# andrewdalpino/UltraZoom

Hardware: AMD Instinct MI355X
Metric: upscaled MPix/sec, MewZoom-4X 1080p bf16 batched inference (higher is better)
Workload: dtype bf16; 1 GPU; MewZoom-4X 96ch/40L bf16, 16 x 1080x1920 -> 4320x7680 per GPU; global_batch=16, parallelism=batch-sharded x1, images_in_flight=0

## Files before the change

ultrazoom_amd/csrc/mz_conv3r.h:

```cpp
#pragma once
#include "mz_device.h"
#include "mz_diag.h"
#include "mz_relay.h"

namespace mz {
namespace r3 {

constexpr int TH = 8;
template <int GEO> struct Geo {
    static_assert(GEO == 0 || GEO == 1, "8 x 48 or 8 x 40");
    static constexpr int TW = GEO == 0 ? 48 : 40;
    static constexpr int NPF = GEO == 0 ? 6 : 5;
    static constexpr int ROWW = TW + 2;
    static constexpr int NPIX = 10 * ROWW;
    static constexpr int DIV_MAGIC = GEO == 0 ? 1311 : 1561;
    static constexpr int X0 = 3, X1 = NPF - 3;
    static constexpr bool straddle(int pf) { return GEO == 1 && pf == 2; }
    static constexpr int dy(int pf) { return GEO == 0 ? pf / 3 : (pf >= 3 ? 1 : 0); }
    static constexpr int dx(int pf) { return GEO == 0 ? 16 * (pf % 3) : (pf < 2 ? 16 * pf : (pf == 2 ? 0 : 8 + 16 * (pf - 3))); }
};
constexpr int PLANE_ENT = 512;
constexpr int A_PLANE = PLANE_ENT * 16;
constexpr int A_SLOT = 4 * A_PLANE;
constexpr int NT = 3, NF = 6, BN = 96;
constexpr int NG = 9 * NT;
constexpr int B_BASE = 2 * A_SLOT;
constexpr int CHUNK_PIECES = 2 * NG;
constexpr int MIX_PIECES = 4 * NT * NT;

template <int NSEG> struct Seg {
    static_assert(NSEG == 2 || NSEG == 3, "two or three weight segments per chunk");
    static constexpr int start(int s) { return NSEG == 2 ? (s <= 0 ? 0 : (s == 1 ? (NG + 1) / 2 : NG)) : (NG / 3) * s; }
    static constexpr int of(int G) { return NSEG == 2 ? (G < start(1) ? 0 : 1) : G / (NG / 3); }
    static constexpr int pieces(int s) { return 2 * (start(s + 1) - start(s)); }
    static constexpr int SLOT = pieces(0) * 1024;
    static constexpr int MIX_BASE = B_BASE + 3 * SLOT;
    static constexpr int lds_bytes(bool fuse) { return fuse ? MIX_BASE + MIX_PIECES * 1024 : B_BASE + 3 * SLOT; }
};

template <int GEO, int TAP, int PF> constexpr int a_off() {
    using GG = Geo<GEO>;
    constexpr int DY = TAP / 3, DX = TAP % 3;
    return ((DY + GG::dy(PF)) * GG::ROWW + DX + GG::dx(PF)) * 16;
}

template <int NPF> struct Frag {
    u32x4 x[2][NPF];
    u32x4 w[3][2];
};

template <int N> __device__ __forceinline__ void wait_w(u32x4& w0, u32x4& w1) {
    asm volatile("s_waitcnt lgkmcnt(%2)" : "+v"(w0), "+v"(w1) : "n"(N) : "memory");
}
template <int N>
__device__ __forceinline__ void wait_wx(u32x4& w0, u32x4& w1, u32x4 (&x)[6]) {
    asm volatile("s_waitcnt lgkmcnt(%8)"
                 : "+v"(w0), "+v"(w1), "+v"(x[0]), "+v"(x[1]), "+v"(x[2]), "+v"(x[3]), "+v"(x[4]), "+v"(x[5])
                 : "n"(N)
                 : "memory");
}
template <int N>
__device__ __forceinline__ void wait_wx(u32x4& w0, u32x4& w1, u32x4 (&x)[5]) {
    asm volatile("s_waitcnt lgkmcnt(%7)"
                 : "+v"(w0), "+v"(w1), "+v"(x[0]), "+v"(x[1]), "+v"(x[2]), "+v"(x[3]), "+v"(x[4])
                 : "n"(N)
                 : "memory");
}

struct Bases {
    uint32_t a_cur, a_nxt, b_cur, b_nxt;
    uint32_t a2_cur, a2_nxt;
};
template <int GEO, int TAP, int PF> __device__ __forceinline__ u32x4 read_x(const Bases& bs, const bool next_image) {
    if constexpr (Geo<GEO>::straddle(PF)) return lds_read128<a_off<GEO, TAP, PF>()>(next_image ? bs.a2_nxt : bs.a2_cur);
    else return lds_read128<a_off<GEO, TAP, PF>()>(next_image ? bs.a_nxt : bs.a_cur);
}

template <class TT, int NSEG, int GEO, int GC, int XP, bool ZERO_C, int M>
__device__ __forceinline__ void group_mfmas(f32x4 (&acc)[Geo<GEO>::NPF][NF], Frag<Geo<GEO>::NPF>& f, const Bases& bs) {
    using GG = Geo<GEO>;
    constexpr int NPF = GG::NPF;
    if constexpr (M < 2 * NPF) {
        using S = Seg<NSEG>;
        constexpr int t = GC / 3, n = GC % 3, xp = (t + XP) & 1, xq = xp ^ 1;
        constexpr int sg = S::of(GC);
        constexpr int Gs = S::start(sg), Ge = S::start(sg + 1);
        constexpr int T = GC + 2;
        constexpr bool t_here = T < Ge;
        constexpr int t_idx = t_here ? T - Gs : T - Ge;
        constexpr int pf = (n & 1) ? NPF - 1 - M / 2 : M / 2, k = ((M / 2) & 1) ? 1 - (M & 1) : (M & 1);
        if constexpr (ZERO_C) mma16_first<TT>(acc[pf][2 * n + k], f.w[GC % 3][k], f.x[xp][pf]);
        else mma16<TT>(acc[pf][2 * n + k], f.w[GC % 3][k], f.x[xp][pf]);
        __builtin_amdgcn_sched_barrier(0);
        if constexpr (M < 2) {
            f.w[T % 3][M] = lds_read128<(2 * t_idx + M) * 1024>(t_here ? bs.b_cur : bs.b_nxt);
            __builtin_amdgcn_sched_barrier(0);
        }
        if constexpr (n < 2 && M >= 2 && M < 2 + (n == 0 ? GG::X0 : GG::X1)) {
            constexpr int pfn = GG::X0 * n + (M - 2);
            if constexpr (t + 1 < 9) f.x[xq][pfn] = read_x<GEO, (t + 1 < 9 ? t + 1 : 0), pfn>(bs, false);
            else f.x[xq][pfn] = read_x<GEO, 0, pfn>(bs, true);
            __builtin_amdgcn_sched_barrier(0);
        }
        group_mfmas<TT, NSEG, GEO, GC, XP, ZERO_C, M + 1>(acc, f, bs);
    }
}

template <class TT, int NSEG, int GEO, int G, int GE, int XP>
__device__ __forceinline__ void groups(f32x4 (&acc)[Geo<GEO>::NPF][NF], Frag<Geo<GEO>::NPF>& f, const Bases& bs, bool first) {
    using GG = Geo<GEO>;
    if constexpr (G < GE) {
        constexpr int t = G / 3, n = G % 3;
        __builtin_amdgcn_sched_barrier(0);
        if constexpr (G < 3 && XP == 0) {
            if (first) group_mfmas<TT, NSEG, GEO, G, XP, true, 0>(acc, f, bs);
            else group_mfmas<TT, NSEG, GEO, G, XP, false, 0>(acc, f, bs);
        } else {
            group_mfmas<TT, NSEG, GEO, G, XP, false, 0>(acc, f, bs);
        }
        constexpr int wn = (G + 1) % 3, xn = (t + 1 + XP) & 1;
        if constexpr (n == 2)
            wait_wx<2>(f.w[wn][0], f.w[wn][1], f.x[xn]);
        else if constexpr (n == 1)
            wait_w<GG::X0 + 2 + GG::X1>(f.w[wn][0], f.w[wn][1]);
        else
            wait_w<2 + GG::X0>(f.w[wn][0], f.w[wn][1]);
        groups<TT, NSEG, GEO, G + 1, GE, XP>(acc, f, bs, first);
    }
}

template <int H, int I> __device__ __forceinline__ void gate_reads(u32x4 (&wv)[NT], uint32_t addr) {
    if constexpr (I < NT) {
        constexpr int ks = H >> 1, part = H & 1;
        wv[I] = lds_read128<(ks * 2 * NT + part * NT + I) * 1024>(addr);
        gate_reads<H, I + 1>(wv, addr);
    }
}
template <int N> __device__ __forceinline__ void gate_wait(u32x4 (&wv)[NT]) {
    asm volatile("s_waitcnt lgkmcnt(%3)" : "+v"(wv[0]), "+v"(wv[1]), "+v"(wv[2]) : "n"(N) : "memory");
}
template <class TT, int H>
__device__ __forceinline__ void gate_halves(f32x4 (&beta)[NF], const u32x4 (&xf)[NT], const u32x4 (&zf)[NT], u32x4 (&wa)[NT],
                                            u32x4 (&wb)[NT], uint32_t addr) {
    if constexpr (H < 4 * NT) {
        constexpr int ks = H >> 1, part = H & 1;
        constexpr bool more = H + 1 < 4 * NT;
        if constexpr (more) gate_reads<H + 1, 0>(wb, addr);
        gate_wait<(more ? NT : 0)>(wa);
        __builtin_amdgcn_sched_barrier(0);
#pragma unroll
        for (int i = 0; i < NT; ++i) {
            if constexpr (ks == 0) mma16_first<TT>(beta[part * NT + i], wa[i], xf[0]);
            else if constexpr (ks < NT) mma16<TT>(beta[part * NT + i], wa[i], xf[ks]);
            else mma16<TT>(beta[part * NT + i], wa[i], zf[ks - NT]);
        }
        __builtin_amdgcn_sched_barrier(0);
        gate_halves<TT, H + 1>(beta, xf, zf, wb, wa, addr);
    }
}

}

template <class TT, int NSEG, int EPI, bool SILU, int GEO = 0, bool RAG = false>
__global__ __launch_bounds__(512) void conv3r_kernel(const ConvArgs a) {
    using namespace r3;
    using namespace relay;
    using S = Seg<NSEG>;
    using GG = Geo<GEO>;
    constexpr int NPF = GG::NPF, TW = GG::TW, ROWW = GG::ROWW, NPIX = GG::NPIX;
    constexpr int NE = NPF * NT;
    constexpr bool FUSE = EPI == EPI_FUSEDMIX;
    static_assert(!FUSE || GEO == 0, "the fused variant is built for the 8 x 48 tile");
    constexpr int B_SLOT = S::SLOT;
    static_assert(!FUSE || NSEG == 3, "the gate weights need the LDS that three weight segments leave free");
    static_assert(!RAG || (NSEG == 3 && EPI == EPI_STORE && GEO == 0), "the ragged two-chunk variant: three steps per chunk, plain stores, 8 x 48 tiles");
    extern __shared__ __attribute__((aligned(16))) char smem[];
    const int w = __builtin_amdgcn_readfirstlane((int)threadIdx.x >> 6);
    const int team = w >> 2, wq = w & 3;
    const int nchunks = a.nchunks16;
    const uint32_t lds_base = (uint32_t)(uintptr_t)(__attribute__((address_space(3))) char*)smem;

    const int xcd = blockIdx.x & 7, pos = blockIdx.x >> 3, step = gridDim.x >> 3;
    const int q = a.grid >> 3, rem = a.grid & 7;
    const int cnt = q + (xcd < rem ? 1 : 0);
    const int base = xcd < rem ? xcd * (q + 1) : rem * (q + 1) + (xcd - rem) * q;
    if (pos >= cnt) return;
    typedef uint32_t TabE __attribute__((ext_vector_type(2)));
    typedef const __attribute__((address_space(4))) TabE* TabPtr;
    const TabPtr tab = (TabPtr)(uintptr_t)a.tile_tab + base;
    struct TileE { uint32_t yx, bn; };
    auto tile_at = [&](int i) __attribute__((always_inline)) {
        const TabE e = tab[i];
        return TileE{e[0], e[1]};
    };
    int a_pos = pos;
    TileE eD, eA, eB;
    auto advance = [&]() __attribute__((always_inline)) { a_pos += step; };
    auto tile_origin = [&](const TileE e, int& b, int& y0, int& x0) __attribute__((always_inline)) {
        b = (int)(e.bn & 0xffffu);
        y0 = (int)(e.yx & 0xffffu);
        x0 = (int)(e.yx >> 16);
    };
    auto tile_nt = [](const TileE e) __attribute__((always_inline)) { return (int)(e.bn >> 16); };

    int hs = 0, us = 0;
    auto next3 = [](int v) __attribute__((always_inline)) { return v == 2 ? 0 : v + 1; };

    f32x4 acc[NPF][NF];
    Frag<NPF> f;
    RS_DECL;

    const size_t chunk_bytes = (size_t)CHUNK_PIECES * 1024;
    const long long plane_in = (long long)a.H * a.W * 16;

    uint32_t hoff[2];
    const char* img_l = nullptr;
    auto set_load_tile = [&](const TileE e) __attribute__((always_inline)) {
        int b, y0, x0;
        tile_origin(e, b, y0, x0);
        img_l = (const char*)a.in0 + (long long)b * a.p0 * plane_in;
        const int lane_ = lane_now();
        const bool interior = y0 >= 1 && x0 >= 1 && y0 + TH + 2 <= a.H && x0 + TW + 1 <= a.W;
        const uint32_t delta = ((uint32_t)(y0 - 1) * (uint32_t)a.W + (uint32_t)(x0 - 1)) * 16u;
#pragma unroll
        for (int j = 0; j < 2; ++j) {
            const int p = 64 * (wq + 4 * j) + lane_;
            const int py = (p * GG::DIV_MAGIC) >> 16, px = p - py * ROWW;
            uint32_t o = ((uint32_t)py * (uint32_t)a.W + (uint32_t)px) * 16u + delta;
            if (!interior) {
                const int gy = y0 - 1 + py, gx = x0 - 1 + px;
                const bool ok = (p < NPIX) & (gy >= 0) & (gy < a.H) & (gx >= 0) & (gx < a.W);
                o = ok ? o : 0xffffffffu;
            }
            hoff[j] = o;
        }
    };
    auto halo_piece = [&](auto i_tag, const __amdgpu_buffer_rsrc_t rsrc, char* dst, [[maybe_unused]] const bool rag = false) __attribute__((always_inline)) {
        constexpr int i = decltype(i_tag)::value;
        uint32_t off = hoff[i & 1];
        if constexpr (RAG) {
            if (rag && (i >> 1) >= a.ragged_planes) off = 0xffffffffu;
        }
        __builtin_amdgcn_raw_ptr_buffer_load_lds(rsrc, (__attribute__((address_space(3))) void*)(dst + (wq + 4 * i) * 1024), 16,
                                                 (int)off, (int)((uint32_t)(i >> 1) * (uint32_t)plane_in), 0, 0);
    };
    auto halo_rsrc = [&](int kc) __attribute__((always_inline)) {
        return __builtin_amdgcn_make_buffer_rsrc((void*)(img_l + 4LL * kc * plane_in), 0, (int)(uint32_t)(4 * plane_in), 0x00020000);
    };
    auto wseg_count = [&](int pieces) __attribute__((always_inline)) { return pieces > wq ? (pieces - wq + 3) >> 2 : 0; };
    auto wseg_piece = [&](auto i_tag, const char* s0, int mine, char* dst, uint32_t lo) __attribute__((always_inline)) {
        constexpr int i = decltype(i_tag)::value;
        if (i < mine) glds16(s0 + (size_t)wq * 1024u + (size_t)i * 4096u + lo, dst + wq * 1024 + i * 4096);
    };
    constexpr int WP = (S::pieces(0) + 3) / 4;
    auto wsrc_of = [&](int nt) __attribute__((always_inline)) {
        return (const char*)a.wpk16 + (size_t)nt * nchunks * chunk_bytes;
    };

    __amdgpu_buffer_rsrc_t orsrc;
    u32x4 xrsrc = {0u, 0u, 0u, 0u};
    uint32_t x_lane = 0;
    uint32_t e_pix = 0, eoff[NT] = {0, 0, 0};
    int e_c = 0, e_y = 0;
    [[maybe_unused]] int e_sdy = 0, e_sdx = 0;
    [[maybe_unused]] uint32_t e_soff = 0;
    auto epi_setup = [&]() __attribute__((always_inline)) {
        const int lane_ = lane_now();
        const int g = lane_ >> 4, c = lane_ & 15;
        const int lane_cu = 2 * (g & 1) + (g >> 1);
        int d_b, d_y0, d_x0;
        tile_origin(eD, d_b, d_y0, d_x0);
        const int d_nbase = tile_nt(eD) * BN;
        e_c = d_x0 + c;
        e_y = d_y0 + 2 * wq;
        if constexpr (GEO == 1) {
            e_sdy = c >= 8 ? 1 : 0;
            e_sdx = c >= 8 ? -8 : 32;
        }
        if constexpr (EPI == EPI_D2S) {
            const long long plane_o = (long long)a.Hout * a.Wout * 16;
            orsrc = __builtin_amdgcn_make_buffer_rsrc((char*)a.out + (long long)d_b * a.p_out * plane_o, 0,
                                                      (int)(uint32_t)(a.p_out * plane_o), 0x00020000);
            e_pix = ((uint32_t)(2 * e_y) * (uint32_t)a.Wout + (uint32_t)(2 * e_c)) * 16u;
            if constexpr (GEO == 1) e_soff = (uint32_t)((2 * e_sdy * a.Wout + 2 * e_sdx) * 16);
#pragma unroll
            for (int n = 0; n < NT; ++n) {
                const int nch = d_nbase + (4 * n + lane_cu) * 8;
                const int ij = nch / a.cp_out, ch = nch - ij * a.cp_out;
                eoff[n] = nch < 4 * a.cp_out
                              ? (uint32_t)(ch >> 3) * (uint32_t)plane_o + ((uint32_t)(ij >> 1) * (uint32_t)a.Wout + (uint32_t)(ij & 1)) * 16u
                              : 0xffffffffu;
            }
        } else {
            const long long plane_o = (long long)a.H * a.W * 16;
            const int p_first = d_nbase >> 3;
            const int planes = a.p_out - p_first < 4 * NT ? a.p_out - p_first : 4 * NT;
            orsrc = __builtin_amdgcn_make_buffer_rsrc((char*)a.out + ((long long)d_b * a.p_out + p_first) * plane_o, 0,
                                                      (int)(uint32_t)(planes * plane_o), 0x00020000);
            e_pix = ((uint32_t)e_y * (uint32_t)a.W + (uint32_t)e_c) * 16u;
            if constexpr (GEO == 1) e_soff = (uint32_t)((e_sdy * a.W + e_sdx) * 16);
#pragma unroll
            for (int n = 0; n < NT; ++n) eoff[n] = (uint32_t)(4 * n + lane_cu) * (uint32_t)plane_o;
            if constexpr (FUSE) {
                const unsigned long long xb = (unsigned long long)(uintptr_t)((const char*)a.in1 + (long long)d_b * a.p1 * plane_o);
                xrsrc[0] = (uint32_t)__builtin_amdgcn_readfirstlane((int)(uint32_t)xb);
                xrsrc[1] = (uint32_t)__builtin_amdgcn_readfirstlane((int)(uint32_t)((xb >> 32) & 0xffffu));
                xrsrc[2] = (uint32_t)__builtin_amdgcn_readfirstlane((int)(uint32_t)(a.p1 * plane_o));
                xrsrc[3] = 0x00020000u;
                x_lane = (uint32_t)(g >> 1) * (uint32_t)plane_o + (uint32_t)(g & 1) * 8u;
            }
        }
    };
    typedef uint32_t u32x2_ __attribute__((ext_vector_type(2)));
    u32x2_ f_xq[2][NF];
    u32x4 f_zb[NT];
    auto entry_words = [&](auto e_tag, u32x4& o) __attribute__((always_inline)) {
        constexpr int E = decltype(e_tag)::value;
        constexpr int pf = E / NT, n = E % NT;
        uint32_t pa[2], pb[2];
#pragma unroll
        for (int h = 0; h < 2; ++h) {
            float a0 = acc[pf][2 * n][2 * h], a1 = acc[pf][2 * n][2 * h + 1], b0 = acc[pf][2 * n + 1][2 * h], b1 = acc[pf][2 * n + 1][2 * h + 1];
            if constexpr (FUSE) {
                float xa[2], za[2], xc[2], zc[2];
                unpack2r<TT>(f_xq[pf & 1][2 * n][h], xa[0], xa[1]);
                unpack2r<TT>(f_zb[n][h], za[0], za[1]);
                unpack2r<TT>(f_xq[pf & 1][2 * n + 1][h], xc[0], xc[1]);
                unpack2r<TT>(f_zb[n][2 + h], zc[0], zc[1]);
                blend_pair_to(a0, a1, acc[pf][2 * n][2 * h], acc[pf][2 * n][2 * h + 1], xa[0], xa[1], za[0], za[1], a.inv_mix_scale);
                blend_pair_to(b0, b1, acc[pf][2 * n + 1][2 * h], acc[pf][2 * n + 1][2 * h + 1], xc[0], xc[1], zc[0], zc[1], a.inv_mix_scale);
            }
            if constexpr (EPI == EPI_STORE && SILU) {
                silu_pair_to(a0, a1, acc[pf][2 * n][2 * h], acc[pf][2 * n][2 * h + 1]);
                silu_pair_to(b0, b1, acc[pf][2 * n + 1][2 * h], acc[pf][2 * n + 1][2 * h + 1]);
            }
            pa[h] = pack_pair<TT>(f32x2{a0, a1});
            pb[h] = pack_pair<TT>(f32x2{b0, b1});
        }
        o = swap_packed(pa, pb);
    };
    auto epi_store = [&](auto e_tag, const u32x4& o) __attribute__((always_inline)) {
        constexpr int E = decltype(e_tag)::value;
        constexpr int pf = E / NT, n = E % NT;
        bool inside;
        uint32_t off;
        if constexpr (GG::straddle(pf)) {
            inside = e_y + e_sdy < a.H && e_c + e_sdx < a.W;
            off = e_pix + e_soff + eoff[n];
        } else {
            inside = e_y + GG::dy(pf) < a.H && e_c + GG::dx(pf) < a.W;
            if constexpr (EPI == EPI_D2S) off = e_pix + (uint32_t)(2 * GG::dy(pf)) * (uint32_t)a.Wout * 16u + (uint32_t)(2 * GG::dx(pf)) * 16u + eoff[n];
            else off = e_pix + (uint32_t)GG::dy(pf) * (uint32_t)a.W * 16u + (uint32_t)GG::dx(pf) * 16u + eoff[n];
        }
        if (!inside || eoff[n] == 0xffffffffu) off = 0xffffffffu;
        __builtin_amdgcn_raw_buffer_store_b128(o, orsrc, (int)off, 0, 0);
    };
    auto fuse_x = [&](auto pf_tag) __attribute__((always_inline)) {
        constexpr int pf = decltype(pf_tag)::value;
        const bool inside = e_y + GG::dy(pf) < a.H && e_c + GG::dx(pf) < a.W;
        const long long plane_o = (long long)a.H * a.W * 16;
        uint32_t off = e_pix + (uint32_t)GG::dy(pf) * (uint32_t)a.W * 16u + (uint32_t)GG::dx(pf) * 16u + x_lane;
        if (!inside) off = 0xffffffffu;
#pragma unroll
        for (int nf = 0; nf < NF; ++nf) {
            const uint32_t o = inside ? off + (uint32_t)(2 * nf) * (uint32_t)plane_o : 0xffffffffu;
            u32x2_& dst = f_xq[pf & 1][nf];
            const u32x4& xr = xrsrc;
            asm volatile("buffer_load_dwordx2 %0, %1, %2, 0 offen" : "=v"(dst) : "v"(o), "s"(xr) : "memory");
        }
    };
    auto x_landed = [&](auto pf_tag) __attribute__((always_inline)) {
        constexpr int pf = decltype(pf_tag)::value;
#pragma unroll
        for (int nf = 0; nf < NF; ++nf) {
            u32x2_& r = f_xq[pf & 1][nf];
            asm volatile("" : "+v"(r));
        }
    };
    auto fuse_z = [&](auto pf_tag) __attribute__((always_inline)) {
        constexpr int pf = decltype(pf_tag)::value;
#pragma unroll
        for (int m = 0; m < NT; ++m) {
            const f32x4 za = acc[pf][2 * m], zc = acc[pf][2 * m + 1];
            u32x4 q;
            q[0] = pack2r<TT>(za[0], za[1]); q[1] = pack2r<TT>(za[2], za[3]);
            q[2] = pack2r<TT>(zc[0], zc[1]); q[3] = pack2r<TT>(zc[2], zc[3]);
            asm volatile("" : "+v"(q));
            f_zb[m] = q;
        }
    };
    auto fuse_a = [&](auto pf_tag) __attribute__((always_inline)) {
        constexpr int pf = decltype(pf_tag)::value;
        if constexpr (pf + 1 < NPF) fuse_x(ic<(pf + 1 < NPF ? pf + 1 : 0)>{});
        fuse_z(pf_tag);
    };
    auto fuse_c = [&](auto pf_tag) __attribute__((always_inline)) {
        constexpr int pf = decltype(pf_tag)::value;
        const int lane_ = lane_now();
        const uint32_t mix_lane = lds_base + S::MIX_BASE + lane_ * 16;
        u32x4 xb[NT];
#pragma unroll
        for (int m = 0; m < NT; ++m) xb[m] = u32x4{f_xq[pf & 1][2 * m][0], f_xq[pf & 1][2 * m][1], f_xq[pf & 1][2 * m + 1][0], f_xq[pf & 1][2 * m + 1][1]};
        u32x4 wa[NT], wb[NT];
        gate_reads<0, 0>(wa, mix_lane);
        gate_halves<TT, 0>(acc[pf], xb, f_zb, wa, wb, mix_lane);
        gate_settle();
    };
    auto entry_whole = [&](auto e_tag) __attribute__((always_inline)) {
        if constexpr (decltype(e_tag)::value < NE) {
            u32x4 o;
            entry_words(e_tag, o);
            epi_store(e_tag, o);
        }
    };

    auto prime = [&](int wslot, int aslot) __attribute__((always_inline)) {
        const int lane_ = lane_now();
        const int g = lane_ >> 4, c = lane_ & 15;
        Bases pb;
        pb.a_cur = pb.a_nxt = lds_base + aslot * A_SLOT + g * A_PLANE + ((2 * wq) * ROWW + c) * 16;
        pb.a2_cur = pb.a2_nxt = pb.a_cur + (uint32_t)((c >= 8 ? ROWW - 8 : 32) * 16);
        pb.b_cur = pb.b_nxt = 0;
        const uint32_t bb = lds_base + B_BASE + wslot * B_SLOT + lane_ * 16;
        f.x[0][0] = read_x<GEO, 0, 0>(pb, false);
        f.x[0][1] = read_x<GEO, 0, 1>(pb, false);
        f.x[0][2] = read_x<GEO, 0, 2>(pb, false);
        f.x[0][3] = read_x<GEO, 0, 3>(pb, false);
        f.x[0][4] = read_x<GEO, 0, 4>(pb, false);
        if constexpr (NPF > 5) f.x[0][NPF - 1] = read_x<GEO, 0, NPF - 1>(pb, false);
        f.w[0][0] = lds_read128<0 * 1024>(bb);
        f.w[0][1] = lds_read128<1 * 1024>(bb);
        f.w[1][0] = lds_read128<2 * 1024>(bb);
        f.w[1][1] = lds_read128<3 * 1024>(bb);
        wait_wx<0>(f.w[0][0], f.w[0][1], f.x[0]);
        wait_w<0>(f.w[1][0], f.w[1][1]);
    };

    const char* wA = nullptr;
    const char* wB = nullptr;
    bool okB = false;
    auto loader_step = [&](auto wk_tag, auto es_tag, auto en_tag, auto sg_tag, auto last_tag, int k) __attribute__((always_inline)) {
        constexpr int WK = decltype(wk_tag)::value;
        constexpr int ES = decltype(es_tag)::value, EN = WK == 0 ? 0 : decltype(en_tag)::value, sg = decltype(sg_tag)::value;
        constexpr bool last = decltype(last_tag)::value != 0;
        [[maybe_unused]] constexpr int rs_c = 1 + (EN > 0 ? 2 : 0) + (sg == 0 ? 0 : 1);
        static_assert(EN <= 3, "three output registers");
        constexpr int VM_AFTER0 = WK == 1 ? EN : (WK == 2 ? (ES + 1 < NPF ? NF : 0) : (WK == 4 ? EN * NT : 0));
        constexpr int VM_AFTER = VM_AFTER0 + (NSEG == 3 && sg == 0 ? 8 : 0);
        RS_BEGIN();
        if constexpr (WK == 2 && ES == 0) fuse_x(ic<0>{});
        if constexpr (WK == 3) x_landed(ic<ES>{});
        constexpr bool HALO_LATE = NSEG == 3;
        auto halo_image = [&]() __attribute__((always_inline)) {
            const __amdgpu_buffer_rsrc_t h_rsrc = halo_rsrc(last ? 0 : k + 1);
            uint32_t h_off = (uint32_t)(us ^ 1) * (uint32_t)A_SLOT;
            asm volatile("" : "+s"(h_off));
            char* const h_dst = smem + h_off;
            const bool rag = RAG && !last && k + 2 == nchunks;
            halo_piece(ic<0>{}, h_rsrc, h_dst, rag); halo_piece(ic<1>{}, h_rsrc, h_dst, rag); halo_piece(ic<2>{}, h_rsrc, h_dst, rag);
            halo_piece(ic<3>{}, h_rsrc, h_dst, rag); halo_piece(ic<4>{}, h_rsrc, h_dst, rag); halo_piece(ic<5>{}, h_rsrc, h_dst, rag);
            halo_piece(ic<6>{}, h_rsrc, h_dst, rag); halo_piece(ic<7>{}, h_rsrc, h_dst, rag);
        };
        if constexpr (sg == 0 && !HALO_LATE) {
            if (!last || okB) halo_image();
        }
        {
            constexpr bool same = sg + 2 < NSEG;
            constexpr int qs = same ? sg + 2 : sg + 2 - NSEG;
            const char* wsrc;
            bool w_ok = true;
            if constexpr (same) wsrc = wA + (size_t)k * chunk_bytes;
            else if constexpr (!last) wsrc = wA + (size_t)(k + 1) * chunk_bytes;
            else { wsrc = wB; w_ok = okB; }
            wsrc += (size_t)(2 * S::start(qs)) * 1024;
            const int w_pieces = w_ok ? wseg_count(S::pieces(qs)) : 0;
            char* const w_dst = smem + B_BASE + (hs >= 1 ? hs - 1 : 2) * B_SLOT;
            const uint32_t lo = (uint32_t)lane_now() * 16u;
            wseg_piece(ic<0>{}, wsrc, w_pieces, w_dst, lo); wseg_piece(ic<1>{}, wsrc, w_pieces, w_dst, lo); wseg_piece(ic<2>{}, wsrc, w_pieces, w_dst, lo);
            wseg_piece(ic<3>{}, wsrc, w_pieces, w_dst, lo); wseg_piece(ic<4>{}, wsrc, w_pieces, w_dst, lo);
            if constexpr (WP > 5) wseg_piece(ic<5>{}, wsrc, w_pieces, w_dst, lo);
            if constexpr (WP > 6) wseg_piece(ic<6>{}, wsrc, w_pieces, w_dst, lo);
            static_assert(WP <= 7, "seven weight pieces per wave and step");
        }
        if constexpr (sg == 0 && HALO_LATE) halo_image();
        __builtin_amdgcn_sched_barrier(0);
        asm volatile("" ::: "memory");
        RS_LAP(4 * rs_c);
        if constexpr (WK == 1) {
            u32x4 o0, o1, o2;
            if constexpr (EN > 0) entry_words(ic<ES>{}, o0);
            if constexpr (EN > 1) entry_words(ic<ES + 1>{}, o1);
            if constexpr (EN > 2) entry_words(ic<ES + 2>{}, o2);
            if constexpr (EN > 0) epi_store(ic<ES>{}, o0);
            if constexpr (EN > 1) epi_store(ic<ES + 1>{}, o1);
            if constexpr (EN > 2) epi_store(ic<ES + 2>{}, o2);
        } else if constexpr (WK == 2) {
            static_assert(WK != 2 || EN == 1, "one pixel fragment per chunk");
            fuse_a(ic<ES>{});
        } else if constexpr (WK == 3) {
            fuse_c(ic<ES>{});
        } else if constexpr (WK == 4) {
            entry_whole(ic<3 * ES>{}); entry_whole(ic<3 * ES + 1>{}); entry_whole(ic<3 * ES + 2>{});
        }
        RS_FENCE();
        RS_LAP(4 * rs_c + 1);
        if constexpr (sg == NSEG - 1) {
            if constexpr (last) {
                if constexpr (FUSE) zero_acc(acc);
                prime(next3(hs), us ^ 1);
            } else {
                if (k + 2 == nchunks && okB) {
                    set_load_tile(eB);
                }
            }
        }
        __builtin_amdgcn_sched_barrier(0);
        RS_LAP(sg == NSEG - 1 ? (last ? 26 : 25) : 4 * rs_c + 1);
        wait_vmcnt<VM_AFTER>();
        RS_LAP(4 * rs_c + 2);
        __builtin_amdgcn_s_barrier();
        RS_LAP(4 * rs_c + 3);
        RS_COUNT(20 + rs_c);
        hs = next3(hs);
        if constexpr (sg == NSEG - 1) us ^= 1;
    };
    auto loader_chunk = [&](auto e0_tag, auto n0_tag, auto n1_tag, auto last_tag, int k) __attribute__((always_inline)) {
        constexpr int E0 = decltype(e0_tag)::value < NE ? decltype(e0_tag)::value : NE;
        constexpr int N0 = decltype(n0_tag)::value < NE - E0 ? decltype(n0_tag)::value : NE - E0;
        constexpr int N1 = decltype(n1_tag)::value < NE - E0 - N0 ? decltype(n1_tag)::value : NE - E0 - N0;
        if constexpr (NSEG == 2) {
            loader_step(ic<(N0 > 0)>{}, ic<E0>{}, ic<N0>{}, ic<0>{}, last_tag, k);
            loader_step(ic<(N1 > 0)>{}, ic<E0 + N0>{}, ic<N1>{}, ic<1>{}, last_tag, k);
        } else {
            constexpr int N1a = N1 / 2, N1b = N1 - N1a;
            loader_step(ic<(N0 > 0)>{}, ic<E0>{}, ic<N0>{}, ic<0>{}, last_tag, k);
            loader_step(ic<(N1a > 0)>{}, ic<E0 + N0>{}, ic<N1a>{}, ic<1>{}, last_tag, k);
            loader_step(ic<(N1b > 0)>{}, ic<E0 + N0 + N1a>{}, ic<N1b>{}, ic<2>{}, last_tag, k);
        }
    };
    auto fuse_chunk = [&](auto p0_tag, auto g_tag, auto last_tag, int k) __attribute__((always_inline)) {
        static_assert(!FUSE || NSEG == 3, "the fused variant runs three steps per chunk");
        loader_step(ic<2>{}, p0_tag, g_tag, ic<0>{}, last_tag, k);
        loader_step(ic<3>{}, p0_tag, g_tag, ic<1>{}, last_tag, k);
        loader_step(ic<4>{}, p0_tag, g_tag, ic<NSEG - 1>{}, last_tag, k);
    };
    auto plain_chunks = [&](int k0) __attribute__((always_inline)) {
        for (int k = k0; k + 1 < nchunks; ++k) loader_chunk(ic<0>{}, ic<0>{}, ic<0>{}, ic<0>{}, k);
        loader_chunk(ic<0>{}, ic<0>{}, ic<0>{}, ic<1>{}, nchunks - 1);
    };
    auto loader_phase = [&](auto epi_tag) __attribute__((always_inline)) {
        constexpr bool DO_EPI = decltype(epi_tag)::value != 0;
        wA = wsrc_of(tile_nt(eA));
        okB = a_pos + step < cnt;
        wB = wsrc_of(tile_nt(okB ? eB : eA));
        const TileE eA2 = tile_at(a_pos + 2 * step), eB2 = tile_at(a_pos + 3 * step);
        if constexpr (DO_EPI) {
            RS_BEGIN();
            set_load_tile(eA);
            epi_setup();
            RS_FENCE();
            RS_LAP(27);
            if constexpr (RAG) {
                loader_chunk(ic<0>{}, ic<3>{}, ic<6>{}, ic<0>{}, 0);
                loader_chunk(ic<9>{}, ic<3>{}, ic<6>{}, ic<1>{}, 1);
            } else if constexpr (FUSE) {
                fuse_chunk(ic<0>{}, ic<1>{}, ic<0>{}, 0);
                fuse_chunk(ic<1>{}, ic<1>{}, ic<0>{}, 1);
                fuse_chunk(ic<2>{}, ic<1>{}, ic<0>{}, 2);
                fuse_chunk(ic<3>{}, ic<1>{}, ic<0>{}, 3);
                fuse_chunk(ic<4>{}, ic<1>{}, ic<0>{}, 4);
                if (nchunks == 6) {
                    fuse_chunk(ic<5>{}, ic<1>{}, ic<1>{}, 5);
                } else {
                    fuse_chunk(ic<5>{}, ic<1>{}, ic<0>{}, 5);
                    plain_chunks(6);
                }
            } else if (nchunks >= 6) {
                loader_chunk(ic<0>{}, ic<1>{}, ic<2>{}, ic<0>{}, 0);
                loader_chunk(ic<3>{}, ic<1>{}, ic<2>{}, ic<0>{}, 1);
                loader_chunk(ic<6>{}, ic<1>{}, ic<2>{}, ic<0>{}, 2);
                loader_chunk(ic<9>{}, ic<1>{}, ic<2>{}, ic<0>{}, 3);
                loader_chunk(ic<12>{}, ic<1>{}, ic<2>{}, ic<0>{}, 4);
                if (nchunks == 6) {
                    loader_chunk(ic<15>{}, ic<1>{}, ic<2>{}, ic<1>{}, 5);
                } else {
                    loader_chunk(ic<15>{}, ic<1>{}, ic<2>{}, ic<0>{}, 5);
                    plain_chunks(6);
                }
            } else {
                constexpr int F3 = NSEG == 3 ? 2 : 3;
                loader_chunk(ic<0>{}, ic<F3>{}, ic<6 - F3>{}, ic<0>{}, 0);
                loader_chunk(ic<6>{}, ic<F3>{}, ic<6 - F3>{}, ic<0>{}, 1);
                if (nchunks == 3) {
                    loader_chunk(ic<12>{}, ic<F3>{}, ic<6 - F3>{}, ic<1>{}, 2);
                } else {
                    loader_chunk(ic<12>{}, ic<F3>{}, ic<6 - F3>{}, ic<0>{}, 2);
                    plain_chunks(3);
                }
            }
        } else {
            plain_chunks(0);
        }
        eD = eB; eA = eA2; eB = eB2;
        asm volatile("" ::"s"(eA.yx), "s"(eA.bn), "s"(eB.yx), "s"(eB.bn));
    };

    auto compute_phase = [&]() __attribute__((always_inline)) {
        const int lane_ = lane_now();
        const int g = lane_ >> 4, c = lane_ & 15;
        const uint32_t a_lane = lds_base + g * A_PLANE + ((2 * wq) * ROWW + c) * 16;
        Bases bs;
        bs.a_cur = a_lane + us * A_SLOT;
        bs.a_nxt = a_lane + (us ^ 1) * A_SLOT;
        const uint32_t a_str = (uint32_t)((c >= 8 ? ROWW - 8 : 32) * 16);
        bs.a2_cur = bs.a_cur + a_str;
        bs.a2_nxt = bs.a_nxt + a_str;
        const uint32_t bl = lds_base + B_BASE + lane_ * 16;
        uint32_t b0 = bl + hs * B_SLOT, b1 = bl + next3(hs) * B_SLOT, b2 = bl + next3(next3(hs)) * B_SLOT;
        bs.b_cur = b0;
        bs.b_nxt = b1;
        auto step_tail = [&]() __attribute__((always_inline)) {
            __builtin_amdgcn_s_barrier();
            const uint32_t u_ = b0; b0 = b1; b1 = b2; b2 = u_;
            bs.b_cur = b0; bs.b_nxt = b1;
        };
        auto chunk = [&](auto xp_tag, bool first) __attribute__((always_inline)) {
            constexpr int XP = decltype(xp_tag)::value;
            groups<TT, NSEG, GEO, S::start(0), S::start(1), XP>(acc, f, bs, first);
            step_tail();
            groups<TT, NSEG, GEO, S::start(1), S::start(2), XP>(acc, f, bs, false);
            step_tail();
            if constexpr (NSEG == 3) {
                groups<TT, NSEG, GEO, S::start(2), S::start(3), XP>(acc, f, bs, false);
                step_tail();
            }
            const uint32_t v_ = bs.a_cur; bs.a_cur = bs.a_nxt; bs.a_nxt = v_;
            if constexpr (GEO == 1) { const uint32_t v2_ = bs.a2_cur; bs.a2_cur = bs.a2_nxt; bs.a2_nxt = v2_; }
        };
        RS_BEGIN();
        int kc = 0;
        for (;;) {
            chunk(ic<0>{}, !FUSE && kc == 0);
            if (++kc >= nchunks) break;
            chunk(ic<1>{}, false);
            if (++kc >= nchunks) break;
        }
        asm volatile("s_waitcnt lgkmcnt(0)"
                     : "+v"(f.x[0][0]), "+v"(f.x[0][1]), "+v"(f.x[0][2]), "+v"(f.x[0][3]), "+v"(f.x[0][4]), "+v"(f.x[0][NPF - 1]),
                       "+v"(f.x[1][0]), "+v"(f.x[1][1]), "+v"(f.x[1][2]), "+v"(f.x[1][3]), "+v"(f.x[1][4]), "+v"(f.x[1][NPF - 1])
                     :
                     : "memory");
        asm volatile("" : "+v"(f.w[0][0]), "+v"(f.w[0][1]), "+v"(f.w[1][0]), "+v"(f.w[1][1]), "+v"(f.w[2][0]), "+v"(f.w[2][1]));
        RS_LAP(0);
        RS_COUNT(1);
        const int adv = (NSEG * nchunks) % 3;
        hs = hs + adv >= 3 ? hs + adv - 3 : hs + adv;
        us ^= nchunks & 1;
    };
    auto final_fuse_pf = [&](auto pf_tag) __attribute__((always_inline)) {
        constexpr int pf = decltype(pf_tag)::value;
        fuse_x(pf_tag);
        fuse_z(pf_tag);
        wait_vmcnt<0>();
        x_landed(pf_tag);
        fuse_c(pf_tag);
        entry_whole(ic<3 * pf>{}); entry_whole(ic<3 * pf + 1>{}); entry_whole(ic<3 * pf + 2>{});
    };
    auto final_epilogue = [&]() __attribute__((always_inline)) {
        epi_setup();
        if constexpr (FUSE) {
            final_fuse_pf(ic<0>{}); final_fuse_pf(ic<1>{}); final_fuse_pf(ic<2>{}); final_fuse_pf(ic<3>{}); final_fuse_pf(ic<4>{}); final_fuse_pf(ic<5>{});
        } else {
            entry_whole(ic<0>{}); entry_whole(ic<1>{}); entry_whole(ic<2>{}); entry_whole(ic<3>{}); entry_whole(ic<4>{}); entry_whole(ic<5>{});
            entry_whole(ic<6>{}); entry_whole(ic<7>{}); entry_whole(ic<8>{}); entry_whole(ic<9>{}); entry_whole(ic<10>{}); entry_whole(ic<11>{});
            entry_whole(ic<12>{}); entry_whole(ic<13>{}); entry_whole(ic<14>{}); entry_whole(ic<15>{}); entry_whole(ic<16>{}); entry_whole(ic<17>{});
        }
    };

    if (team == 1) {
        eA = tile_at(a_pos);
        eB = tile_at(a_pos + step);
        eD = eA;
        wA = wsrc_of(tile_nt(eA));
        set_load_tile(eA);
        {
            const __amdgpu_buffer_rsrc_t r0 = halo_rsrc(0);
            halo_piece(ic<0>{}, r0, smem); halo_piece(ic<1>{}, r0, smem); halo_piece(ic<2>{}, r0, smem); halo_piece(ic<3>{}, r0, smem);
            halo_piece(ic<4>{}, r0, smem); halo_piece(ic<5>{}, r0, smem); halo_piece(ic<6>{}, r0, smem); halo_piece(ic<7>{}, r0, smem);
            const char* s1 = wA + (size_t)(2 * S::start(1)) * 1024;
            const uint32_t lo = (uint32_t)lane_now() * 16u;
            char* d0 = smem + B_BASE;
            char* d1 = smem + B_BASE + B_SLOT;
            wseg_piece(ic<0>{}, wA, wseg_count(S::pieces(0)), d0, lo); wseg_piece(ic<1>{}, wA, wseg_count(S::pieces(0)), d0, lo); wseg_piece(ic<2>{}, wA, wseg_count(S::pieces(0)), d0, lo);
            wseg_piece(ic<3>{}, wA, wseg_count(S::pieces(0)), d0, lo); wseg_piece(ic<4>{}, wA, wseg_count(S::pieces(0)), d0, lo); wseg_piece(ic<5>{}, wA, wseg_count(S::pieces(0)), d0, lo);
            wseg_piece(ic<6>{}, wA, wseg_count(S::pieces(0)), d0, lo);
            wseg_piece(ic<0>{}, s1, wseg_count(S::pieces(1)), d1, lo); wseg_piece(ic<1>{}, s1, wseg_count(S::pieces(1)), d1, lo); wseg_piece(ic<2>{}, s1, wseg_count(S::pieces(1)), d1, lo);
            wseg_piece(ic<3>{}, s1, wseg_count(S::pieces(1)), d1, lo); wseg_piece(ic<4>{}, s1, wseg_count(S::pieces(1)), d1, lo); wseg_piece(ic<5>{}, s1, wseg_count(S::pieces(1)), d1, lo);
            wseg_piece(ic<6>{}, s1, wseg_count(S::pieces(1)), d1, lo);
        }
        if constexpr (FUSE) {
            const int lane_ = lane_now();
            const char* msrc = (const char*)a.wmix16 + (uint32_t)lane_ * 16u;
#pragma unroll
            for (int i = 0; i < MIX_PIECES / 4; ++i) glds16(msrc + (size_t)(wq + 4 * i) * 1024, smem + S::MIX_BASE + (wq + 4 * i) * 1024);
        }
        wait_vmcnt<0>();
        __builtin_amdgcn_s_barrier();
        if constexpr (FUSE) zero_acc(acc);
        loader_phase(ic<0>{});
        advance();
        if (a_pos >= cnt) { RS_DUMP(); return; }
    } else {
        eD = tile_at(a_pos);
        eA = tile_at(a_pos + step);
        eB = tile_at(a_pos + 2 * step);
        asm volatile("" ::"s"(eD.yx), "s"(eD.bn), "s"(eA.yx), "s"(eA.bn), "s"(eB.yx), "s"(eB.bn));
        __builtin_amdgcn_s_barrier();
        if constexpr (FUSE) zero_acc(acc);
        prime(0, 0);
    }
    for (;;) {
        compute_phase();
        advance();
        if (a_pos >= cnt) {
            RS_BEGIN();
            final_epilogue();
            RS_LAP(2);
            RS_DUMP();
            return;
        }
        loader_phase(ic<1>{});
        advance();
        if (a_pos >= cnt) { RS_DUMP(); return; }
    }
}

}
```

ultrazoom_amd/csrc/mz_diag.h:

```cpp
#pragma once
#ifdef MZ_DIAG
#define RS_DECL                                                                                              \
    uint32_t rs_[32] = {};                                                                                   \
    uint32_t rs_t0 = 0, rs_t1 = 0;                                                                           \
    unsigned long long rs_c0, rs_r0;                                                                         \
    asm volatile("s_memtime %0\n\ts_memrealtime %1\n\ts_waitcnt lgkmcnt(0)" : "=s"(rs_c0), "=s"(rs_r0)::"memory")
#define RS_NOW(v)                                                                         \
    do {                                                                                  \
        unsigned long long t__;                                                           \
        asm volatile("s_memtime %0\n\ts_waitcnt lgkmcnt(0)" : "=s"(t__)::"memory");       \
        v = (uint32_t)t__;                                                                \
    } while (0)
#define RS_BEGIN() RS_NOW(rs_t0)
#define RS_LAP(i)                 \
    do {                          \
        RS_NOW(rs_t1);            \
        rs_[i] += rs_t1 - rs_t0;  \
        rs_t0 = rs_t1;            \
    } while (0)
#define RS_COUNT(i) do { rs_[i] += 1; } while (0)
#define RS_FENCE() __builtin_amdgcn_sched_barrier(0)
#define RS_DUMP()                                                                                              \
    do {                                                                                                       \
        unsigned long long rs_c1, rs_r1;                                                                       \
        asm volatile("s_memtime %0\n\ts_memrealtime %1\n\ts_waitcnt lgkmcnt(0)" : "=s"(rs_c1), "=s"(rs_r1)::"memory"); \
        rs_[28] = (uint32_t)(rs_c1 - rs_c0);                          \
        rs_[29] = (uint32_t)(rs_r1 - rs_r0);                                        \
        if (a.dbg && blockIdx.x == gridDim.x / 2 && (threadIdx.x & 63) == 0) {                                               \
            _Pragma("unroll") for (int i__ = 0; i__ < 32; ++i__) a.dbg[w * 32 + i__] = rs_[i__];              \
        }                                                                                                      \
    } while (0)
#else
#define RS_DECL do { } while (0)
#define RS_BEGIN() do { } while (0)
#define RS_LAP(i) do { } while (0)
#define RS_COUNT(i) do { } while (0)
#define RS_FENCE() do { } while (0)
#define RS_DUMP() do { } while (0)
#endif
```

Measured before the change: 711.4 MPix/s.

## Spread fused gate MFMAs and output stores across loader steps

Reorders the fused-mix gate GEMM into units of three fragments indexed per output pair, so the gate work can be split. In the fused kernel the whole gate for a pixel fragment now runs in the earlier loader step, and part of the output stores move forward into the following step. The goal is to balance work between steps and hide load latency. The final epilogue also prefetches the next fragment's x before waiting, with a relaxed vmcnt, instead of draining all loads. Diagnostic counters are extended to cover the new step. The risk is more register pressure and subtle wait-count mistakes.

```diff
diff --git a/ultrazoom_amd/csrc/mz_conv3r.h b/ultrazoom_amd/csrc/mz_conv3r.h
--- a/ultrazoom_amd/csrc/mz_conv3r.h
+++ b/ultrazoom_amd/csrc/mz_conv3r.h
@@ -129,33 +129,38 @@
     }
 }
 
-template <int H, int I> __device__ __forceinline__ void gate_reads(u32x4 (&wv)[NT], uint32_t addr) {
+template <int U, int I> __device__ __forceinline__ void gate_reads(u32x4 (&wv)[NT], uint32_t addr) {
     if constexpr (I < NT) {
-        constexpr int ks = H >> 1, part = H & 1;
-        wv[I] = lds_read128<(ks * 2 * NT + part * NT + I) * 1024>(addr);
-        gate_reads<H, I + 1>(wv, addr);
+        constexpr int n = U >> 2, j = NT * (U & 3) + I, ks = j >> 1, k = j & 1;
+        wv[I] = lds_read128<(ks * 2 * NT + 2 * n + k) * 1024>(addr);
+        gate_reads<U, I + 1>(wv, addr);
     }
 }
 template <int N> __device__ __forceinline__ void gate_wait(u32x4 (&wv)[NT]) {
     asm volatile("s_waitcnt lgkmcnt(%3)" : "+v"(wv[0]), "+v"(wv[1]), "+v"(wv[2]) : "n"(N) : "memory");
 }
-template <class TT, int H>
-__device__ __forceinline__ void gate_halves(f32x4 (&beta)[NF], const u32x4 (&xf)[NT], const u32x4 (&zf)[NT], u32x4 (&wa)[NT],
-                                            u32x4 (&wb)[NT], uint32_t addr) {
-    if constexpr (H < 4 * NT) {
-        constexpr int ks = H >> 1, part = H & 1;
-        constexpr bool more = H + 1 < 4 * NT;
-        if constexpr (more) gate_reads<H + 1, 0>(wb, addr);
+template <class TT, int U, int I>
+__device__ __forceinline__ void gate_unit_mfmas(f32x4 (&beta)[NF], const u32x4 (&xf)[NT], const u32x4 (&zf)[NT], const u32x4 (&wv)[NT]) {
+    if constexpr (I < NT) {
+        constexpr int n = U >> 2, j = NT * (U & 3) + I, ks = j >> 1, k = j & 1;
+        if constexpr (ks == 0) mma16_first<TT>(beta[2 * n + k], wv[I], xf[0]);
+        else if constexpr (ks < NT) mma16<TT>(beta[2 * n + k], wv[I], xf[ks]);
+        else mma16<TT>(beta[2 * n + k], wv[I], zf[ks - NT]);
+        gate_unit_mfmas<TT, U, I + 1>(beta, xf, zf, wv);
+    }
+}
+template <class TT, int U, int UE>
+__device__ __forceinline__ void gate_units(f32x4 (&beta)[NF], const u32x4 (&xf)[NT], const u32x4 (&zf)[NT], u32x4 (&wa)[NT],
+                                           u32x4 (&wb)[NT], uint32_t addr) {
+    static_assert(NT == 3 && UE <= 4 * NT, "four units of three fragments per pair");
+    if constexpr (U < UE) {
+        constexpr bool more = U + 1 < UE;
+        if constexpr (more) gate_reads<U + 1, 0>(wb, addr);
         gate_wait<(more ? NT : 0)>(wa);
         __builtin_amdgcn_sched_barrier(0);
-#pragma unroll
-        for (int i = 0; i < NT; ++i) {
-            if constexpr (ks == 0) mma16_first<TT>(beta[part * NT + i], wa[i], xf[0]);
-            else if constexpr (ks < NT) mma16<TT>(beta[part * NT + i], wa[i], xf[ks]);
-            else mma16<TT>(beta[part * NT + i], wa[i], zf[ks - NT]);
-        }
+        gate_unit_mfmas<TT, U, 0>(beta, xf, zf, wa);
         __builtin_amdgcn_sched_barrier(0);
-        gate_halves<TT, H + 1>(beta, xf, zf, wb, wa, addr);
+        gate_units<TT, U + 1, UE>(beta, xf, zf, wb, wa, addr);
     }
 }
 
@@ -394,18 +399,19 @@
         if constexpr (pf + 1 < NPF) fuse_x(ic<(pf + 1 < NPF ? pf + 1 : 0)>{});
         fuse_z(pf_tag);
     };
-    auto fuse_c = [&](auto pf_tag) __attribute__((always_inline)) {
-        constexpr int pf = decltype(pf_tag)::value;
+    auto fuse_gate = [&](auto pf_tag, auto n0_tag, auto n1_tag) __attribute__((always_inline)) {
+        constexpr int pf = decltype(pf_tag)::value, N0 = decltype(n0_tag)::value, N1 = decltype(n1_tag)::value;
         const int lane_ = lane_now();
         const uint32_t mix_lane = lds_base + S::MIX_BASE + lane_ * 16;
         u32x4 xb[NT];
 #pragma unroll
         for (int m = 0; m < NT; ++m) xb[m] = u32x4{f_xq[pf & 1][2 * m][0], f_xq[pf & 1][2 * m][1], f_xq[pf & 1][2 * m + 1][0], f_xq[pf & 1][2 * m + 1][1]};
         u32x4 wa[NT], wb[NT];
-        gate_reads<0, 0>(wa, mix_lane);
-        gate_halves<TT, 0>(acc[pf], xb, f_zb, wa, wb, mix_lane);
+        gate_reads<4 * N0, 0>(wa, mix_lane);
+        gate_units<TT, 4 * N0, 4 * N1>(acc[pf], xb, f_zb, wa, wb, mix_lane);
         gate_settle();
     };
+    auto fuse_c = [&](auto pf_tag) __attribute__((always_inline)) { fuse_gate(pf_tag, ic<0>{}, ic<NT>{}); };
     auto entry_whole = [&](auto e_tag) __attribute__((always_inline)) {
         if constexpr (decltype(e_tag)::value < NE) {
             u32x4 o;
@@ -443,13 +449,16 @@
         constexpr int WK = decltype(wk_tag)::value;
         constexpr int ES = decltype(es_tag)::value, EN = WK == 0 ? 0 : decltype(en_tag)::value, sg = decltype(sg_tag)::value;
         constexpr bool last = decltype(last_tag)::value != 0;
-        [[maybe_unused]] constexpr int rs_c = 1 + (EN > 0 ? 2 : 0) + (sg == 0 ? 0 : 1);
+        [[maybe_unused]] constexpr int rs_c = WK == 4 ? 5 : 1 + (EN > 0 ? 2 : 0) + (sg == 0 ? 0 : 1);
+        [[maybe_unused]] constexpr int rs_b = rs_c < 5 ? 4 * rs_c : 32, rs_n = rs_c < 5 ? 20 + rs_c : 36;
         static_assert(EN <= 3, "three output registers");
-        constexpr int VM_AFTER0 = WK == 1 ? EN : (WK == 2 ? (ES + 1 < NPF ? NF : 0) : (WK == 4 ? EN * NT : 0));
+        [[maybe_unused]] constexpr bool SPREAD = FUSE && ES >= 1;
+        [[maybe_unused]] constexpr int GA = NT, EC = 2;
+        constexpr int VM_AFTER0 = WK == 1 ? EN : (WK == 2 ? (ES + 1 < NPF ? NF : 0) : (WK == 3 ? (SPREAD ? EC : 0) : (WK == 4 ? (SPREAD ? NT - EC : NT) : 0)));
         constexpr int VM_AFTER = VM_AFTER0 + (NSEG == 3 && sg == 0 ? 8 : 0);
         RS_BEGIN();
         if constexpr (WK == 2 && ES == 0) fuse_x(ic<0>{});
-        if constexpr (WK == 3) x_landed(ic<ES>{});
+        if constexpr (WK == 3 && !SPREAD) x_landed(ic<ES>{});
         constexpr bool HALO_LATE = NSEG == 3;
         auto halo_image = [&]() __attribute__((always_inline)) {
             const __amdgpu_buffer_rsrc_t h_rsrc = halo_rsrc(last ? 0 : k + 1);
@@ -485,7 +494,7 @@
         if constexpr (sg == 0 && HALO_LATE) halo_image();
         __builtin_amdgcn_sched_barrier(0);
         asm volatile("" ::: "memory");
-        RS_LAP(4 * rs_c);
+        RS_LAP(rs_b);
         if constexpr (WK == 1) {
             u32x4 o0, o1, o2;
             if constexpr (EN > 0) entry_words(ic<ES>{}, o0);
@@ -497,13 +506,26 @@
         } else if constexpr (WK == 2) {
             static_assert(WK != 2 || EN == 1, "one pixel fragment per chunk");
             fuse_a(ic<ES>{});
+            if constexpr (SPREAD) {
+                x_landed(ic<ES>{});
+                fuse_gate(ic<ES>{}, ic<0>{}, ic<GA>{});
+            }
         } else if constexpr (WK == 3) {
-            fuse_c(ic<ES>{});
+            if constexpr (SPREAD) {
+                if constexpr (GA < NT) fuse_gate(ic<ES>{}, ic<GA>{}, ic<NT>{});
+                if constexpr (EC > 0) entry_whole(ic<3 * ES>{});
+                if constexpr (EC > 1) entry_whole(ic<3 * ES + 1>{});
+                if constexpr (EC > 2) entry_whole(ic<3 * ES + 2>{});
+            } else {
+                fuse_c(ic<ES>{});
+            }
         } else if constexpr (WK == 4) {
-            entry_whole(ic<3 * ES>{}); entry_whole(ic<3 * ES + 1>{}); entry_whole(ic<3 * ES + 2>{});
+            if constexpr (!SPREAD || EC < 1) entry_whole(ic<3 * ES>{});
+            if constexpr (!SPREAD || EC < 2) entry_whole(ic<3 * ES + 1>{});
+            if constexpr (!SPREAD || EC < 3) entry_whole(ic<3 * ES + 2>{});
         }
         RS_FENCE();
-        RS_LAP(4 * rs_c + 1);
+        RS_LAP(rs_b + 1);
         if constexpr (sg == NSEG - 1) {
             if constexpr (last) {
                 if constexpr (FUSE) zero_acc(acc);
@@ -515,12 +537,12 @@
             }
         }
         __builtin_amdgcn_sched_barrier(0);
-        RS_LAP(sg == NSEG - 1 ? (last ? 26 : 25) : 4 * rs_c + 1);
+        RS_LAP(sg == NSEG - 1 ? (last ? 26 : 25) : rs_b + 1);
         wait_vmcnt<VM_AFTER>();
-        RS_LAP(4 * rs_c + 2);
+        RS_LAP(rs_b + 2);
         __builtin_amdgcn_s_barrier();
-        RS_LAP(4 * rs_c + 3);
-        RS_COUNT(20 + rs_c);
+        RS_LAP(rs_b + 3);
+        RS_COUNT(rs_n);
         hs = next3(hs);
         if constexpr (sg == NSEG - 1) us ^= 1;
     };
@@ -659,9 +681,10 @@
     };
     auto final_fuse_pf = [&](auto pf_tag) __attribute__((always_inline)) {
         constexpr int pf = decltype(pf_tag)::value;
-        fuse_x(pf_tag);
+        if constexpr (pf == 0) fuse_x(pf_tag);
+        if constexpr (pf + 1 < NPF) fuse_x(ic<(pf + 1 < NPF ? pf + 1 : 0)>{});
         fuse_z(pf_tag);
-        wait_vmcnt<0>();
+        wait_vmcnt<(pf + 1 < NPF ? NF : 0) + (pf > 0 ? NT : 0)>();
         x_landed(pf_tag);
         fuse_c(pf_tag);
         entry_whole(ic<3 * pf>{}); entry_whole(ic<3 * pf + 1>{}); entry_whole(ic<3 * pf + 2>{});
diff --git a/ultrazoom_amd/csrc/mz_diag.h b/ultrazoom_amd/csrc/mz_diag.h
--- a/ultrazoom_amd/csrc/mz_diag.h
+++ b/ultrazoom_amd/csrc/mz_diag.h
@@ -1,7 +1,7 @@
 #pragma once
 #ifdef MZ_DIAG
 #define RS_DECL                                                                                              \
-    uint32_t rs_[32] = {};                                                                                   \
+    uint32_t rs_[40] = {};                                                                                   \
     uint32_t rs_t0 = 0, rs_t1 = 0;                                                                           \
     unsigned long long rs_c0, rs_r0;                                                                         \
     asm volatile("s_memtime %0\n\ts_memrealtime %1\n\ts_waitcnt lgkmcnt(0)" : "=s"(rs_c0), "=s"(rs_r0)::"memory")
@@ -28,6 +28,8 @@
         rs_[29] = (uint32_t)(rs_r1 - rs_r0);                                        \
         if (a.dbg && blockIdx.x == gridDim.x / 2 && (threadIdx.x & 63) == 0) {                                               \
             _Pragma("unroll") for (int i__ = 0; i__ < 32; ++i__) a.dbg[w * 32 + i__] = rs_[i__];              \
+             \
+            _Pragma("unroll") for (int i__ = 32; i__ < 40; ++i__) a.dbg[256 + w * 8 + i__ - 32] = rs_[i__];   \
         }                                                                                                      \
     } while (0)
 #else
```

Result: no change. 713.7 MPix/s, median of 6 (+0.3%).
